# EDIpack/EDIpack

Measured on AMD Instinct MI355X. Metric: Lanczos H*v iterations/sec, largest (Nup,Ndw) sector, higher is better.
Workload: dtype f64

## Files before the change

edipack_amd/csrc/edigpu_capi.hip:

```cpp
#include <algorithm>
#include <chrono>
#include <cmath>
#include <cstdlib>
#include <cstring>
#include <map>
#include <memory>
#include <mutex>
#include <tuple>

#include "host_ib.hpp"
#include "host_sb.hpp"
#include "kernels.hpp"

namespace edigpu {

static thread_local std::string g_err;
static thread_local int g_device = 0;
void set_error(const std::string& msg) { g_err = msg; }

template <class T>
static int dev_upload(T** d, const T* h, size_t n) {
  *d = nullptr;
  if (n == 0) return 0;
  EDIGPU_HIP(hipMalloc((void**)d, n * sizeof(T)));
  EDIGPU_HIP(hipMemcpy(*d, h, n * sizeof(T), hipMemcpyHostToDevice));
  return 0;
}

template <class T>
static void dev_free(T*& p) {
  if (p) (void)hipFree(p);
  p = nullptr;
}

static int ensure_device(int* count_out = nullptr) {
  int n = 0;
  hipError_t e = hipGetDeviceCount(&n);
  if (e != hipSuccess || n <= 0) {
    set_error(std::string("edigpu: no usable HIP device (") +
              (e != hipSuccess ? hipGetErrorString(e) : "device count 0") +
              "); this library has no CPU fallback");
    if (count_out) *count_out = 0;
    return 1;
  }
  if (count_out) *count_out = n;
  return 0;
}

static int upload_csr(DevCsr& d, int64_t nrow, const int64_t* rowptr, const int32_t* col,
                      const double* val, int cplx) {
  d = DevCsr();
  d.nrow = nrow;
  d.nnz = rowptr ? rowptr[nrow] : 0;
  d.avg_row = nrow > 0 ? (double)d.nnz / (double)nrow : 0.0;
  if (nrow == 0) return 0;
  if (d.nnz >= ((int64_t)1 << 31)) {
    d.wide = 1;
    if (dev_upload(&d.rowptr64, rowptr, (size_t)nrow + 1)) return 1;
  } else {
    std::vector<int32_t> rp((size_t)nrow + 1);
    for (int64_t i = 0; i <= nrow; i++) rp[i] = (int32_t)rowptr[i];
    if (dev_upload(&d.rowptr32, rp.data(), rp.size())) return 1;
  }
  std::vector<int32_t> cpad(col, col + d.nnz);
  cpad.resize((size_t)d.nnz + 8, 0);
  std::vector<double> vpad(val, val + (size_t)d.nnz * (cplx ? 2 : 1));
  vpad.resize(vpad.size() + 8, 0.0);
  if (dev_upload(&d.col, cpad.data(), cpad.size())) return 1;
  if (dev_upload(&d.val, vpad.data(), vpad.size())) return 1;
  return 0;
}

static void free_ell(DevEll& e) {
  dev_free(e.pk);
  dev_free(e.coef);
  dev_free(e.col);
  dev_free(e.val);
}

static void free_csr(DevCsr& d) {
  dev_free(d.sell_ptr);
  dev_free(d.sell_pk);
  dev_free(d.sell_dict);
  dev_free(d.sell_diag);
  dev_free(d.sell_col);
  dev_free(d.sell_val);
  dev_free(d.rowptr32);
  dev_free(d.rowptr64);
  dev_free(d.col);
  dev_free(d.val);
}

static int upload_ell(DevEll& e, const HostCsr& a, bool lds) {
  e = DevEll();
  const uint32_t cmul = lds ? 8u : 1u;
  e.nrow = a.nrow;
  e.pitch = (a.nrow + 63) / 64 * 64;
  int w = 0;
  for (int64_t i = 0; i < a.nrow; i++) w = std::max<int>(w, (int)(a.rowptr[i + 1] - a.rowptr[i]));
  e.width = w;
  if (w == 0 || a.nrow == 0) return 0;
  std::vector<double> coef(1, 0.0);
  bool packable = (a.nrow + 1) * (int64_t)cmul < ((int64_t)1 << 24);
  std::vector<uint8_t> cid((size_t)a.nnz());
  for (int64_t p = 0; p < a.nnz() && packable; p++) {
    const double m = std::fabs(a.val[p]);
    size_t k = 0;
    for (; k < coef.size(); k++)
      if (coef[k] == m) break;
    if (k == coef.size()) {
      if (coef.size() >= 128) {
        packable = false;
        break;
      }
      coef.push_back(m);
    }
    cid[p] = (uint8_t)k;
  }
  bool typed = packable && coef.size() > 1 && !getenv("EDIGPU_ELL_UNTYPED");
  std::vector<int> maxmult(coef.size(), 0), base(coef.size() + 1, 0);
  if (typed) {
    std::vector<int> cnt(coef.size());
    for (int64_t i = 0; i < a.nrow; i++) {
      std::fill(cnt.begin(), cnt.end(), 0);
      for (int64_t p = a.rowptr[i]; p < a.rowptr[i + 1]; p++) cnt[cid[p]]++;
      for (size_t v = 1; v < coef.size(); v++) maxmult[v] = std::max(maxmult[v], cnt[v]);
    }
    for (size_t v = 1; v < coef.size(); v++) base[v + 1] = base[v] + maxmult[v];
    const int nt = base[coef.size()];
    typed = nt >= 1 && nt <= 127 && nt <= std::max(2 * w, w + 8);
  }
  if (typed) {
    const int nt = base[coef.size()];
    e.width = nt;
    e.typed = 1;
    std::vector<double> tc(128, 0.0);
    for (size_t v = 1; v < coef.size(); v++)
      for (int j = 0; j < maxmult[v]; j++) tc[base[v] + j] = coef[v];
    std::vector<uint32_t> pk((size_t)nt * e.pitch, lds ? (uint32_t)a.nrow * 8u : 0u);
    std::vector<int> occ(coef.size());
    for (int64_t i = 0; i < a.nrow; i++) {
      std::fill(occ.begin(), occ.end(), 0);
      for (int64_t p = a.rowptr[i]; p < a.rowptr[i + 1]; p++) {
        if (cid[p] == 0) continue;
        const int slot = base[cid[p]] + occ[cid[p]]++;
        pk[(size_t)slot * e.pitch + i] = (uint32_t)a.col[p] * cmul | (lds ? 0u : 1u << 24) |
                                         (std::signbit(a.val[p]) ? 0x80000000u : 0u);
      }
    }
    if (dev_upload(&e.pk, pk.data(), pk.size())) return 1;
    if (dev_upload(&e.coef, tc.data(), tc.size())) return 1;
    return 0;
  }
  if (packable) {
    coef.resize(128, 0.0);
    std::vector<uint32_t> pk((size_t)w * e.pitch);
    for (int k = 0; k < w; k++)
      for (int64_t i = 0; i < e.pitch; i++) pk[(size_t)k * e.pitch + i] = (uint32_t)std::min(i, a.nrow - 1) * cmul;
    for (int64_t i = 0; i < a.nrow; i++) {
      int k = 0;
      for (int64_t p = a.rowptr[i]; p < a.rowptr[i + 1]; p++, k++)
        pk[(size_t)k * e.pitch + i] = (uint32_t)a.col[p] * cmul | ((uint32_t)cid[p] << 24) |
                                      (std::signbit(a.val[p]) ? 0x80000000u : 0u);
    }
    if (dev_upload(&e.pk, pk.data(), pk.size())) return 1;
    if (dev_upload(&e.coef, coef.data(), coef.size())) return 1;
    return 0;
  }
  std::vector<int32_t> col((size_t)w * e.pitch);
  std::vector<double> val((size_t)w * e.pitch, 0.0);
  for (int k = 0; k < w; k++)
    for (int64_t i = 0; i < e.pitch; i++) col[(size_t)k * e.pitch + i] = (int32_t)std::min(i, a.nrow - 1);
  for (int64_t i = 0; i < a.nrow; i++) {
    int k = 0;
    for (int64_t p = a.rowptr[i]; p < a.rowptr[i + 1]; p++, k++) {
      col[(size_t)k * e.pitch + i] = a.col[p];
      val[(size_t)k * e.pitch + i] = a.val[p];
    }
  }
  if (dev_upload(&e.col, col.data(), col.size())) return 1;
  if (dev_upload(&e.val, val.data(), val.size())) return 1;
  return 0;
}

static int upload_sell(DevCsr& d, int64_t nrow, int64_t ncol, const int64_t* rowptr, const int32_t* col,
                       const double* val, int cplx, bool is_loc, double max_pad = 1.6) {
  if (nrow == 0 || rowptr[nrow] == 0 || getenv("EDIGPU_CSR_NOSELL")) return 0;
  const int w = cplx ? 2 : 1;
  bool packed = ncol < ((int64_t)1 << 24) && !getenv("EDIGPU_CSR_UNPACKED");
  std::vector<double> dict(w, 0.0);
  std::vector<uint8_t> ids;
  std::vector<double> diag;
  if (packed) {
    ids.assign((size_t)rowptr[nrow], 0);
    if (is_loc) diag.assign((size_t)nrow * w, 0.0);
    for (int64_t i = 0; i < nrow && packed; i++)
      for (int64_t k = rowptr[i]; k < rowptr[i + 1]; k++) {
        if (is_loc && col[k] == i) {
          for (int q = 0; q < w; q++) diag[i * w + q] += val[k * w + q];
          continue;
        }
        const size_t n = dict.size() / w;
        size_t id = 0;
        for (; id < n; id++)
// ... 433 lines not shown
      dst.rimg_len = src.rimg_len;
      for (int i = 0; i < 5; i++) {
        dst.ucls[i] = src.ucls[std::min(i, h.norb + 1)];
        dst.rcb[i] = src.rcb[i];
        dst.rcs[i] = src.rcs[i];
      }
      std::vector<uint32_t> m2((size_t)src.npanels * kIbPanel / 2);
      for (size_t i = 0; i < m2.size(); i++) m2[i] = (uint32_t)src.rmap[2 * i] | ((uint32_t)src.rmap[2 * i + 1] << 16);
      rc = dev_upload(&dst.ublist, src.ublist.data(), src.ublist.size()) || dev_upload(&dst.utop, src.utop.data(), src.utop.size()) ||
           dev_upload(&dst.rmap2, m2.data(), m2.size());
    }
    if (rc) {
      free_ib(p);
      return 1;
    }
  }
  s->ib = d.release();
  if (setup_sb(s->ib, hn, h, chunk_rows)) return 1;
  return setup_pos_rows(s, hn, h);
}

static int setup_normal(edigpu_sector* s, int64_t dim_up, int64_t dim_dw, int64_t dw_first,
                        int64_t dw_count, const double* hd, const HostCsr& up, const HostCsr& dw,
                        const int64_t* nd_rowptr, const int32_t* nd_col, const double* nd_val,
                        HostNormal* built = nullptr) {
  s->kind = 0;
  s->is_complex = 0;
  s->device = g_device;
  s->dim_up = dim_up;
  s->dim_dw = dim_dw;
  s->dw_first = dw_first;
  s->dw_count = dw_count;
  s->dim = dim_up * dim_dw;
  s->nloc = dim_up * dw_count;
  s->row_first = dw_first * dim_up;
  s->h_up = up;
  s->h_dw = dw;
  std::vector<int32_t> tile_starts;
  s->rows_per_block = normal_pick_rows_per_block(dim_up, dw_count);
  {
    const char* e = getenv("EDIGPU_ROW_SPLIT");
    int parts = 0;
    if (e) {
      parts = atoi(e);
      if (parts > 1) s->rows_per_block = 0;
    } else if (s->rows_per_block == 0) {
      parts = (int)(((dim_up + 2) * 8 + 140 * 1024 - 1) / (140 * 1024));
    }
    if (s->rows_per_block == 0 && parts > 1 && dim_up >= 4 * parts) {
      if (upload_ell(s->up_ell, up, true)) return 1;
      if (s->up_ell.typed && s->up_ell.pk) {
        s->row_split = parts;
      } else {
        dev_free(s->up_ell.pk);
        dev_free(s->up_ell.coef);
        dev_free(s->up_ell.col);
        dev_free(s->up_ell.val);
      }
    }
  }
  if (s->row_split == 1 && upload_ell(s->up_ell, up, s->rows_per_block != 0)) return 1;
  if (upload_csr(s->dw, dim_dw, dw.rowptr.data(), dw.col.data(), dw.val.data(), 0)) return 1;
  for (int64_t i = 0; i < dim_dw; i++)
    s->dw_maxrow = std::max<int>(s->dw_maxrow, (int)(dw.rowptr[i + 1] - dw.rowptr[i]));
  {
    const char* e;
    const bool vec2_env = !(e = getenv("EDIGPU_PANEL_VEC2")) || atoi(e) != 0;
    const int64_t vec2_min = (e = getenv("EDIGPU_PANEL_VEC2_MIN")) ? atoll(e) : ((int64_t)1 << 21);
    const bool tile_env = !(e = getenv("EDIGPU_PANEL_TILE")) || atoi(e) != 0;
    int rmax = (e = getenv("EDIGPU_TILE_ROWS")) ? atoi(e) : 32;
    if (rmax < 8) rmax = 8;
    if (rmax > 64) rmax = 64;
    if (vec2_env && dim_up >= 2 && dim_up * dw_count >= vec2_min) s->panel_mode = 1;
    if (s->panel_mode == 1 && tile_env && dw_count > 0 && dim_dw < ((int64_t)1 << 24)) {
      std::vector<int32_t> starts;
      plan_tile_chunks(dw, dw_first, dw_count, rmax, starts, s->tile_rows);
      s->tile_nchunks = (int)starts.size() - 1;
      if (dev_upload(&s->d_tile_chunks, starts.data(), starts.size())) return 1;
      tile_starts = starts;
      s->panel_mode = 2;
    }
  }
  s->has_nd = nd_rowptr != nullptr && nd_rowptr[s->nloc] > 0;
  s->nd_nnz = s->has_nd ? nd_rowptr[s->nloc] : 0;
  if (built && !nd_rowptr) {
    s->has_nd = built->has_nd && built->nd_nnz > 0;
    s->nd_nnz = s->has_nd ? built->nd_nnz : 0;
  }
  if (built && built->fac.valid && built->fac.nterms <= 16 && !env_flag("EDIGPU_NORMAL_EXPLICIT")) {
    const HostFactored& f = built->fac;
    s->factored = 1;
    s->fac_nimp = f.nimp;
    s->fac_nterms = f.nterms;
    if (dev_upload(&s->d_eux, f.eux.data(), f.eux.size())) return 1;
    if (dev_upload(&s->d_ed, f.ed.data(), f.ed.size())) return 1;
    if (dev_upload(&s->d_impd, f.impd.data(), f.impd.size())) return 1;
    if (f.nterms > 0) {
      if (dev_upload(&s->d_ndcoef, f.coef.data(), f.coef.size())) return 1;
      if (dev_upload(&s->d_jup, f.jup.data(), f.jup.size())) return 1;
      for (int t = 0; t < f.nterms; t++)
        for (int64_t c = 0; c < dim_up; c++) {
          const uint32_t jt = f.jup[(size_t)t * dim_up + c];
          if (jt != 0xFFFFFFFFu)
            s->col_halo = std::max<int>(s->col_halo, (int)std::llabs((int64_t)(jt & 0x7FFFFFFFu) - c));
        }
      if (dev_upload(&s->d_jdw, f.jdw.data(), f.jdw.size())) return 1;
      if (dim_dw < ((int64_t)1 << 24) && f.nterms < 127) {
        std::vector<int32_t> mp((size_t)dw_count + 1, 0), mc;
        std::vector<double> mv;
        for (int64_t r = 0; r < dw_count; r++) {
// ... 2537 lines not shown
    float ms = 0.f;
    rc |= (hipEventElapsedTime(&ms, ev[2 * k], ev[2 * k + 1]) != hipSuccess);
    hv += ms;
  }
  for (auto& e : ev) (void)hipEventDestroy(e);
  if (rc) {
    if (g_err.empty()) set_error("edigpu_lanczos_bench: HIP failure");
    return 1;
  }
  *ms_wall_per_step = std::chrono::duration<double, std::milli>(t1 - t0).count() / steps;
  *ms_hv_per_launch = hv / steps;
  return 0;
}

int edigpu_destroy(edigpu_handle s) {
  if (!s) return 0;
  (void)hipSetDevice(s->device);
  if (s->stream) {
    (void)hipStreamSynchronize(s->stream);
    (void)hipStreamDestroy(s->stream);
  }
  if (s->sub_s) edigpu_destroy(s->sub_s);
  if (s->sub_a) edigpu_destroy(s->sub_a);
  if (s->sub_d) edigpu_destroy(s->sub_d);
  dev_free(s->d_cz);
  dev_free(s->d_hd);
  dev_free(s->d_gu);
  dev_free(s->d_gd);
  dev_free(s->d_mx_rowptr);
  dev_free(s->d_tile_chunks);
  dev_free(s->d_tile_lbeg);
  if (s->lz_graph) (void)hipGraphExecDestroy(s->lz_graph);
  dev_free(s->d_lzcnt);
  dev_free(s->d_bl_meta);
  dev_free(s->d_bl_lend);
  dev_free(s->d_bl_ent);
  dev_free(s->d_bl_wtab);
  if (s->ib) {
    free_ib(s->ib);
    delete s->ib;
    s->ib = nullptr;
  }
  dev_free(s->d_tl_meta);
  dev_free(s->d_tl_col);
  dev_free(s->d_tl_val);
  dev_free(s->d_mx_col);
  dev_free(s->d_mx_val);
  dev_free(s->d_eux);
  dev_free(s->d_ed);
  dev_free(s->d_impd);
  dev_free(s->d_ndcoef);
  dev_free(s->d_jup);
  dev_free(s->d_jdw);
  dev_free(s->up_ell.pk);
  dev_free(s->up_ell.coef);
  dev_free(s->up_ell.col);
  dev_free(s->up_ell.val);
  free_csr(s->dw);
  free_csr(s->nd);
  free_csr(s->loc);
  free_csr(s->nonloc);
  for (const void* q : {(const void*)s->orbs.ell_col, (const void*)s->orbs.ell_val, (const void*)s->orbs.hd,
                        (const void*)s->orbs.eax, (const void*)s->orbs.impbit, (const void*)s->orbs.xtab})
    if (q) (void)hipFree(const_cast<void*>(q));
  s->orbs = OrbsArgs();
  dev_free(s->d_dir_states);
  dev_free(s->d_dir_offdw);
  dev_free(s->d_dir_rkup);
  dev_free(s->d_dir_terms);
  dev_free(s->d_dir_tests);
  dev_free(s->d_dir_dtab);
  dev_free(s->d_dir_xtab);
  dev_free(s->d_vin);
  dev_free(s->d_vout);
  dev_free(s->d_tmp);
  dev_free(s->d_partial);
  dev_free(s->d_scal);
  delete s;
  return 0;
}

}
```

edipack_amd/csrc/edigpu_internal.hpp:

```cpp
#pragma once
#include <hip/hip_runtime.h>

#include <cstdint>
#include <cstdio>
#include <string>
#include <vector>

#include "../../include/edigpu.h"
#include "host_build.hpp"

namespace edigpu {

void set_error(const std::string& msg);

#define EDIGPU_HIP(call)                                                                     \
  do {                                                                                       \
    hipError_t _e = (call);                                                                  \
    if (_e != hipSuccess) {                                                                  \
      ::edigpu::set_error(std::string(#call) + " failed: " + hipGetErrorString(_e) + " (" +  \
                          __FILE__ + ":" + std::to_string(__LINE__) + ")");                  \
      return 1;                                                                              \
    }                                                                                        \
  } while (0)

struct DevCsr {
  int64_t nrow = 0, nnz = 0;
  int wide = 0;
  int32_t* rowptr32 = nullptr;
  int64_t* rowptr64 = nullptr;
  int32_t* col = nullptr;
  double* val = nullptr;
  double avg_row = 0.0;
  int sell = 0;
  int64_t nslice = 0;
  int32_t* sell_ptr = nullptr;
  int32_t* sell_col = nullptr;
  double* sell_val = nullptr;
  int sell_packed = 0;
  uint32_t* sell_pk = nullptr;
  double* sell_dict = nullptr;
  double* sell_diag = nullptr;
};

constexpr int kOrbsMaxAxes = 2 * EDIGPU_MAXORB;
struct OrbsArgs {
  int naxes = 0;
  int64_t dim = 0;
  int64_t dims[kOrbsMaxAxes] = {0};
  int64_t stride[kOrbsMaxAxes] = {0};
  int off[kOrbsMaxAxes] = {0};
  int width[kOrbsMaxAxes] = {0};
  int64_t elloff[kOrbsMaxAxes] = {0};
  const int32_t* ell_col = nullptr;
  const double* ell_val = nullptr;
  const double* hd = nullptr;
  const double* eax = nullptr;
  const uint8_t* impbit = nullptr;
  const double* xtab = nullptr;
};

struct DevEll {
  int64_t nrow = 0, pitch = 0;
  int width = 0;
  int typed = 0;
  uint32_t* pk = nullptr;
  double* coef = nullptr;
  int32_t* col = nullptr;
  double* val = nullptr;
};

struct IbDevHalf {
  int panel0 = 0, npanels = 0, nlist = 0, rimg_len = 0;
  int ucls[5] = {0, 0, 0, 0, 0}, rcb[5] = {0, 0, 0, 0, 0}, rcs[5] = {0, 0, 0, 0, 0};
  uint16_t *ublist = nullptr, *utop = nullptr;
  uint32_t* rmap2 = nullptr;
};

struct DevSb {
  int nb0 = 0, nloc = 0, amode = 0, nbw_up = 0, nbw_dw = 0;
  int rows_nt = 0, rows_nbt = 0, rimg_len = 0, rcs = 0;
  size_t rows_lds = 0, cols_lds = 0;
  uint16_t *urank = nullptr, *ublist = nullptr;
  double* ebw = nullptr;
  int32_t* uslot = nullptr;
  uint32_t* rmap2 = nullptr;
  double *up_vtab = nullptr, *up_tloc = nullptr, *e0 = nullptr;
  uint32_t* up_korb = nullptr;
  int lowbits = 0, nchunks = 0, max_chunk_rows = 0, max_chunk_slots = 0, cols_gs = 8;
  int32_t *chunk_row = nullptr, *chunk_slot = nullptr, *cdesc_off = nullptr;
  uint8_t* cdesc = nullptr;
  double *dw_vtab = nullptr, *dw_tloc = nullptr;
  uint32_t* dw_korb = nullptr;
  uint32_t* nd_dw = nullptr;
  int nhalf = 1;
  struct Half {
    int panel0 = 0, npanels = 0;
    uint32_t* ublist32 = nullptr;
    uint8_t* ugap = nullptr;
    int32_t* uslot = nullptr;
    uint32_t* rmap2 = nullptr;
    double* ebw = nullptr;
  } half[2];
};

struct IbDev {
  DevSb* sb = nullptr;
  int nhalf = 1;
  IbDevHalf half[2];
  uint16_t* urank_low = nullptr;
  double top_eps = 0.0;
  int norb = 0, nb_up = 0, nb_dw = 0, npanels = 0, plen = 0, nlist = 0;
  int ucls[5] = {0, 0, 0, 0, 0};
  int lowbits = 0, nchunks = 0, max_chunk_rows = 0, max_chunk_blocks = 0, nterms = 0, nsub = 1;
  int64_t dim_up = 0, dim_dw = 0, ps = 0, len = 0;
  int rows_nt = 0, rows_nbt = 0;
  size_t rows_lds = 0, cols_lds = 0;
  uint16_t *urank = nullptr, *ublist = nullptr;
  uint32_t* rmap2 = nullptr;
  int rcb[5] = {0, 0, 0, 0, 0}, rcs[5] = {0, 0, 0, 0, 0}, rimg_len = 0;
// ... 114 lines not shown
```

edipack_amd/csrc/kernels_normal.hip:

```cpp
#include <cstdlib>
#include <string>

#include "kernels.hpp"
#include "normal_args.hpp"

namespace edigpu {



constexpr int kE = 4;

template <bool VEC>
__device__ inline void load4(const double* __restrict__ base, int64_t i0, const bool* ok, double* out) {
  if (VEC) {
    const double2 a = ok[0] ? *reinterpret_cast<const double2*>(base + i0) : make_double2(0.0, 0.0);
    const double2 b = ok[2] ? *reinterpret_cast<const double2*>(base + i0 + 2) : make_double2(0.0, 0.0);
    out[0] = a.x;
    out[1] = a.y;
    out[2] = b.x;
    out[3] = b.y;
  } else {
#pragma unroll
    for (int e = 0; e < kE; e++) out[e] = ok[e] ? base[i0 + e] : 0.0;
  }
}

typedef const double __attribute__((address_space(3))) lds_cdouble;
__device__ inline double lds_abs_read(uint32_t byte_addr) { return *reinterpret_cast<lds_cdouble*>(byte_addr); }

template <int NT, int TD, bool USE_LDS, bool LOCAL, bool ND, bool PACKED, bool VEC, bool HDF, int FUSE,
          bool SPLIT = false>
__global__ void __launch_bounds__(NT)
    normal_rows_kernel(NormalArgs a, const double* v_local, const double* __restrict__ v_full,
                       double* hv) {
  extern __shared__ double vs[];

  const int64_t DimUp = a.dim_up;
  const int bsh = a.blk_shift;
  const int64_t bps = a.blk_ps;
  auto vix = [&](int64_t row, int64_t col) -> int64_t {
    return bsh ? (col >> bsh) * bps + (row << bsh) + (col & (((int64_t)1 << bsh) - 1)) : row * DimUp + col;
  };
  const int64_t sf = SPLIT ? a.split_first : 0, sc = SPLIT ? a.split_count : DimUp;
  const int S = ((int)sc + 2) & ~1;
  const int rowB = S * 8;
  double* coef_s = vs + (USE_LDS ? TD * S : 0);
  const int64_t r0 = (int64_t)blockIdx.x * TD;
  const int tid = threadIdx.x;
  int nr = TD;
  if (r0 + nr > a.dw_count) nr = (int)(a.dw_count - r0);
  double beta = 0.0, ibeta = 1.0;
  if (FUSE != 0) {
    if (a.scal[SC_STOP] != 0.0) return;
    if (FUSE >= 2) {
      beta = a.scal[SC_BETA];
      ibeta = 1.0 / beta;
    }
  }
  const double alpha = (FUSE == 3) ? a.scal[SC_ALPHA] : 0.0;
  const double* __restrict__ v_src = (FUSE >= 2) ? hv : v_local;

  if (LOCAL && PACKED && tid < 128) coef_s[tid] = a.ell_coef[tid];
  if (LOCAL && USE_LDS) {
    if ((uint32_t)(uintptr_t)(__attribute__((address_space(3))) double*)vs != 0u) __builtin_trap();
    if (tid < TD) vs[tid * S + sc] = 0.0;
    if (VEC) {
      const int64_t n2 = sc >> 1;
      for (int64_t j0 = 0; j0 < n2; j0 += 4 * NT) {
        double2 t[TD][4];
#pragma unroll
        for (int r = 0; r < TD; r++)
#pragma unroll
          for (int u = 0; u < 4; u++) {
            const int64_t j = j0 + tid + u * NT;
            const int rr = r < nr ? r : 0;
            const int64_t jc = 2 * (j < n2 ? j : n2 - 1);
            t[r][u] = *reinterpret_cast<const double2*>(v_src + vix(r0 + rr, sf + jc));
            if (FUSE == 3) {
              const double2 pp = *reinterpret_cast<const double2*>(v_local + vix(r0 + rr, jc));
              t[r][u].x -= alpha * pp.x;
              t[r][u].y -= alpha * pp.y;
            }
            if (FUSE >= 2) {
              t[r][u].x *= ibeta;
              t[r][u].y *= ibeta;
            }
          }
#pragma unroll
        for (int r = 0; r < TD; r++)
#pragma unroll
          for (int u = 0; u < 4; u++) {
            const int64_t j = j0 + tid + u * NT;
            if (r < nr && j < n2) reinterpret_cast<double2*>(vs + r * S)[j] = t[r][u];
          }
      }
    } else {
      for (int64_t j0 = 0; j0 < sc; j0 += 4 * NT) {
        double t[TD][4];
#pragma unroll
        for (int r = 0; r < TD; r++)
#pragma unroll
          for (int u = 0; u < 4; u++) {
            const int64_t j = j0 + tid + u * NT;
            const int rr = r < nr ? r : 0;
            t[r][u] = v_src[vix(r0 + rr, sf + (j < sc ? j : sc - 1))];
            if (FUSE == 3) t[r][u] -= alpha * v_local[vix(r0 + rr, j < DimUp ? j : DimUp - 1)];
            if (FUSE >= 2) t[r][u] *= ibeta;
          }
#pragma unroll
        for (int r = 0; r < TD; r++)
#pragma unroll
          for (int u = 0; u < 4; u++) {
            const int64_t j = j0 + tid + u * NT;
            if (r < nr && j < sc) vs[r * S + j] = t[r][u];
          }
      }
    }
  }
  __syncthreads();

  for (int64_t c0 = 0; c0 < DimUp; c0 += (int64_t)NT * kE) {
    const int64_t col0 = c0 + (int64_t)tid * kE;
    if (col0 >= DimUp) break;
    double acc[TD][kE];
    bool ok[kE];
#pragma unroll
    for (int e = 0; e < kE; e++) {
      ok[e] = col0 + e < DimUp;
#pragma unroll
      for (int r = 0; r < TD; r++) acc[r][e] = 0.0;
    }

    if (LOCAL) {
#pragma unroll
      for (int r = 0; r < TD; r++)
        if (r < nr) {
          double h[kE], x[kE];
          if (HDF) {
            const int64_t g = a.dw_first + r0 + r;
            const double edr = a.ed[g];
            load4<VEC>(a.eux, (int64_t)a.impd[g] * DimUp + col0, ok, h);
#pragma unroll
            for (int e = 0; e < kE; e++) h[e] += edr;
          } else {
            load4<VEC>(a.hd, (r0 + r) * DimUp + col0, ok, h);
          }
          if (USE_LDS && !SPLIT) {
#pragma unroll
            for (int e = 0; e < kE; e++) x[e] = ok[e] ? vs[r * S + col0 + e] : 0.0;
          } else {
            load4<VEC>(v_local, vix(r0 + r, col0), ok, x);
          }
#pragma unroll
          for (int e = 0; e < kE; e++) acc[r][e] = (SPLIT && sf != 0) ? 0.0 : h[e] * x[e];
        }
      constexpr int KU = 4;
      const bool fast = PACKED && USE_LDS && a.ell_typed != 0;
      if (fast) {
        const uint32_t* __restrict__ epk = a.ell_pk + col0;
        const int epitch = (int)a.ell_pitch;
        for (int k0 = 0; k0 < a.ell_w; k0 += KU) {
          uint4 pk4[KU];
          double tk[KU];
#pragma unroll
          for (int u = 0; u < KU; u++) {
            const int k = k0 + u < a.ell_w ? k0 + u : a.ell_w - 1;
            pk4[u] = *reinterpret_cast<const uint4*>(epk + k * epitch);
            tk[u] = coef_s[k0 + u < 127 ? k0 + u : 127];
          }
#pragma unroll
          for (int u = 0; u < KU; u++) {
            const uint32_t p[kE] = {pk4[u].x, pk4[u].y, pk4[u].z, pk4[u].w};
#pragma unroll
            for (int r = 0; r < TD; r++)
              if (TD == 1 || r < nr) {
#pragma unroll
                for (int e = 0; e < kE; e++) {
                  uint32_t off = p[e] & 0xFFFFFFu;
                  if (SPLIT) {
                    const uint32_t rel = off - (uint32_t)(sf * 8);
                    off = rel < (uint32_t)(sc * 8) ? rel : (uint32_t)(sc * 8);
                  }
                  double x = lds_abs_read((uint32_t)(r * rowB) + off);
                  x = __hiloint2double(__double2hiint(x) ^ (int)(p[e] & 0x80000000u), __double2loint(x));
                  acc[r][e] = fma(tk[u], x, acc[r][e]);
                }
              }
          }
        }
      }
      for (int k0 = fast ? a.ell_w : 0; k0 < a.ell_w; k0 += KU) {
        uint4 pk4[KU];
        int4 pc4[KU];
        double2 pw0[KU], pw1[KU];
#pragma unroll
        for (int u = 0; u < KU; u++) {
          const int k = k0 + u < a.ell_w ? k0 + u : a.ell_w - 1;
          const int64_t o = (int64_t)k * a.ell_pitch + col0;
          if (PACKED) {
            pk4[u] = *reinterpret_cast<const uint4*>(a.ell_pk + o);
          } else {
            pc4[u] = *reinterpret_cast<const int4*>(a.ell_col + o);
            pw0[u] = *reinterpret_cast<const double2*>(a.ell_val + o);
            pw1[u] = *reinterpret_cast<const double2*>(a.ell_val + o + 2);
          }
        }
#pragma unroll
        for (int u = 0; u < KU; u++) {
          const bool live = k0 + u < a.ell_w;
          int32_t cc[kE];
          double ww[kE];
          if (PACKED) {
            const uint32_t p[kE] = {pk4[u].x, pk4[u].y, pk4[u].z, pk4[u].w};
            if (a.ell_typed) {
              const double tk = live ? coef_s[k0 + u] : 0.0;
              if (USE_LDS) {
#pragma unroll
                for (int e = 0; e < kE; e++) {
                  cc[e] = (int32_t)(p[e] & 0xFFFFFFu);
                  ww[e] = __hiloint2double(__double2hiint(tk) ^ (int)(p[e] & 0x80000000u), __double2loint(tk));
                }
              } else {
#pragma unroll
                for (int e = 0; e < kE; e++) {
                  cc[e] = (int32_t)(p[e] & 0xFFFFFFu);
                  const double m = ((p[e] >> 24) & 0x7Fu) ? tk : 0.0;
                  ww[e] = (p[e] >> 31) ? -m : m;
                }
              }
            } else {
#pragma unroll
              for (int e = 0; e < kE; e++) {
                cc[e] = (int32_t)(p[e] & 0xFFFFFFu);
                const double m = live ? coef_s[(p[e] >> 24) & 0x7Fu] : 0.0;
                ww[e] = (p[e] >> 31) ? -m : m;
              }
            }
          } else {
            cc[0] = pc4[u].x; cc[1] = pc4[u].y; cc[2] = pc4[u].z; cc[3] = pc4[u].w;
            ww[0] = live ? pw0[u].x : 0.0; ww[1] = live ? pw0[u].y : 0.0;
            ww[2] = live ? pw1[u].x : 0.0; ww[3] = live ? pw1[u].y : 0.0;
          }
#pragma unroll
          for (int r = 0; r < TD; r++)
            if (r < nr) {
#pragma unroll
              for (int e = 0; e < kE; e++) {
                const double x = USE_LDS ? (PACKED ? *reinterpret_cast<const double*>(
                                                         reinterpret_cast<const char*>(vs) + r * rowB + cc[e])
                                                   : vs[r * S + cc[e]])
                                         : v_local[vix(r0 + r, cc[e])];
                acc[r][e] = fma(ww[e], x, acc[r][e]);
              }
            }
        }
      }
    }
    if (ND) {
      if (a.has_nd) {
        int64_t rp[TD][kE + 1];
#pragma unroll
        for (int r = 0; r < TD; r++)
          if (r < nr) {
            const int64_t i0 = (r0 + r) * DimUp + col0;
#pragma unroll
            for (int e = 0; e <= kE; e++) {
              const int64_t i = (e == 0 || ok[e - 1]) ? i0 + e : i0;
              rp[r][e] = a.nd_rp64 ? a.nd_rp64[i] : (int64_t)a.nd_rp32[i];
            }
          }
#pragma unroll
        for (int r = 0; r < TD; r++)
          if (r < nr) {
#pragma unroll
            for (int e = 0; e < kE; e++)
              if (ok[e]) {
                double s = 0.0;
                for (int64_t jj = rp[r][e]; jj < rp[r][e + 1]; jj++)
                  s += a.nd_val[jj] * v_full[a.nd_col[jj]];
                acc[r][e] += s;
              }
          }
      }
    }
#pragma unroll
    for (int r = 0; r < TD; r++)
      if (r < nr) {
        double* dst = hv + vix(r0 + r, col0);
        if (!LOCAL || (SPLIT && sf != 0)) {
          double old[kE];
          load4<VEC>(hv, vix(r0 + r, col0), ok, old);
#pragma unroll
          for (int e = 0; e < kE; e++) acc[r][e] += old[e];
        }
        if (FUSE >= 2) {
          double pold[kE];
          load4<VEC>(v_local, vix(r0 + r, col0), ok, pold);
          double* pdst = (a.xout ? a.xout : const_cast<double*>(v_local)) + vix(r0 + r, col0);
#pragma unroll
          for (int e = 0; e < kE; e++) acc[r][e] -= beta * pold[e];
          if (VEC) {
            if (ok[0]) *reinterpret_cast<double2*>(pdst) = make_double2(vs[r * S + col0], vs[r * S + col0 + 1]);
            if (ok[2]) *reinterpret_cast<double2*>(pdst + 2) = make_double2(vs[r * S + col0 + 2], vs[r * S + col0 + 3]);
          } else {
#pragma unroll
            for (int e = 0; e < kE; e++)
              if (ok[e]) pdst[e] = vs[r * S + col0 + e];
          }
        }
        if (VEC) {
          if (ok[0]) *reinterpret_cast<double2*>(dst) = make_double2(acc[r][0], acc[r][1]);
          if (ok[2]) *reinterpret_cast<double2*>(dst + 2) = make_double2(acc[r][2], acc[r][3]);
        } else {
#pragma unroll
          for (int e = 0; e < kE; e++)
            if (ok[e]) dst[e] = acc[r][e];
        }
      }
  }
}

int normal_pick_rows_per_block(int64_t dim_up, int64_t dw_count) {
  const int64_t row_bytes = ((dim_up + 2) & ~(int64_t)1) * 8;
  if (const char* e = getenv("EDIGPU_ROWS_TD")) {
    const int td = atoi(e);
    if ((td == 1 || td == 2 || td == 4 || td == 8) && td * row_bytes <= 150 * 1024) return td;
  }
  if (row_bytes > 150 * 1024) return 0;
  int td = 1;
  for (int cand : {2, 4, 8}) {
    if (cand * row_bytes > 24 * 1024) break;
    if ((dw_count + cand - 1) / cand < 1024) break;
    td = cand;
  }
  return td;
}

template <int NT, int TD, bool USE_LDS, bool PACKED, bool VEC, bool HDF>
static int launch_te(const NormalArgs& a, const double* vl, const double* vf, double* hv,
                     int what, hipStream_t st) {
  const int64_t nblk = (a.dw_count + TD - 1) / TD;
  const size_t lds = (USE_LDS ? (size_t)TD * ((a.dim_up + 2) & ~(int64_t)1) * sizeof(double) : 0) + 128 * sizeof(double);
  dim3 grid((unsigned)nblk), block(NT);
#define EDIGPU_LAUNCH_ROWS(LOC, NDF, LDSB, UL, PK, HF)                                           \
  do {                                                                                           \
    auto kern = normal_rows_kernel<NT, TD, UL, LOC, NDF, PK, VEC, HF, 0>;                            \
    if (ensure_dynamic_lds((const void*)kern, (LDSB))) return 1; \
    hipLaunchKernelGGL(kern, grid, block, (LDSB), st, a, vl, vf, hv);                            \
  } while (0)
  switch (what) {
    case 1: EDIGPU_LAUNCH_ROWS(true, false, lds, USE_LDS, PACKED, HDF); break;
    case 5: EDIGPU_LAUNCH_ROWS(true, true, lds, USE_LDS, PACKED, HDF); break;
    case 101: {
      auto kern = normal_rows_kernel<NT, TD, USE_LDS, true, false, PACKED, VEC, HDF, 1>;
      if (ensure_dynamic_lds((const void*)kern, lds)) return 1;
      hipLaunchKernelGGL(kern, grid, block, lds, st, a, vl, vf, hv);
      break;
    }
    case 102: {
      auto kern = normal_rows_kernel<NT, TD, USE_LDS, true, false, PACKED, VEC, HDF, 2>;
      if (ensure_dynamic_lds((const void*)kern, lds)) return 1;
      hipLaunchKernelGGL(kern, grid, block, lds, st, a, vl, vf, hv);
      break;
    }
    case 103: {
      auto kern = normal_rows_kernel<NT, TD, USE_LDS, true, false, PACKED, VEC, HDF, 3>;
      if (ensure_dynamic_lds((const void*)kern, lds)) return 1;
      hipLaunchKernelGGL(kern, grid, block, lds, st, a, vl, vf, hv);
      break;
    }
    case 4: EDIGPU_LAUNCH_ROWS(false, true, (size_t)0, false, false, false); break;
    default: set_error("launch_normal: bad term mask"); return 1;
  }
#undef EDIGPU_LAUNCH_ROWS
  EDIGPU_HIP(hipGetLastError());
  return 0;
}

template <int TD, bool USE_LDS>
static int launch_td(const NormalArgs& a, bool packed, bool hdf, const double* vl, const double* vf,
                     double* hv, int what, hipStream_t st) {
  const bool vec = (a.dim_up % 2) == 0;
  const bool big = TD == 1 && USE_LDS && (size_t)a.dim_up * sizeof(double) > 80 * 1024;
  constexpr int NTBIG = (TD == 1 && USE_LDS) ? 1024 : 512;
#define EDIGPU_TD(PK, VC)                                                                  \
  (big ? (hdf ? launch_te<NTBIG, TD, USE_LDS, PK, VC, true>(a, vl, vf, hv, what, st)       \
              : launch_te<NTBIG, TD, USE_LDS, PK, VC, false>(a, vl, vf, hv, what, st))     \
       : (hdf ? launch_te<512, TD, USE_LDS, PK, VC, true>(a, vl, vf, hv, what, st)         \
              : launch_te<512, TD, USE_LDS, PK, VC, false>(a, vl, vf, hv, what, st)))
  if (vec) return packed ? EDIGPU_TD(true, true) : EDIGPU_TD(false, true);
  return packed ? EDIGPU_TD(true, false) : EDIGPU_TD(false, false);
#undef EDIGPU_TD
}

template <bool VEC, bool HDF>
static int launch_split_t(const edigpu_sector* s, NormalArgs a, const double* vl, double* hv, hipStream_t st) {
  constexpr int NT = 1024;
  const int64_t part = (((a.dim_up + s->row_split - 1) / s->row_split) + 1) & ~(int64_t)1;
  auto kern = normal_rows_kernel<NT, 1, true, true, false, true, VEC, HDF, 0, true>;
  const size_t lds = (size_t)((part + 2) & ~(int64_t)1) * sizeof(double) + 128 * sizeof(double);
  if (ensure_dynamic_lds((const void*)kern, lds)) return 1;
  for (int64_t first = 0; first < a.dim_up; first += part) {
    a.split_first = first;
    a.split_count = std::min<int64_t>(part, a.dim_up - first);
    hipLaunchKernelGGL(kern, dim3((unsigned)a.dw_count), dim3(NT), lds, st, a, vl, nullptr, hv);
  }
  EDIGPU_HIP(hipGetLastError());
  return 0;
}

static int launch_rows(const edigpu_sector* s, const NormalArgs& a, const double* vl,
                       const double* vf, double* hv, int what, hipStream_t st) {
  const bool packed = s->up_ell.pk != nullptr;
  const bool hdf = s->factored != 0;
  if (s->row_split > 1 && what != 4) {
    if (what != 1 && what != 5) {
      set_error("launch_normal: fused Lanczos is not available for split rows");
      return 1;
    }
    const bool vec = (a.dim_up % 2) == 0;
    const int rc = vec ? (hdf ? launch_split_t<true, true>(s, a, vl, hv, st) : launch_split_t<true, false>(s, a, vl, hv, st))
                       : (hdf ? launch_split_t<false, true>(s, a, vl, hv, st) : launch_split_t<false, false>(s, a, vl, hv, st));
    if (rc || what == 1) return rc;
    return launch_td<1, false>(a, false, hdf, vl, vf, hv, 4, st);
  }
  switch (s->rows_per_block) {
    case 0: return launch_td<1, false>(a, packed, hdf, vl, vf, hv, what, st);
    case 1: return launch_td<1, true>(a, packed, hdf, vl, vf, hv, what, st);
    case 2: return launch_td<2, true>(a, packed, hdf, vl, vf, hv, what, st);
    case 4: return launch_td<4, true>(a, packed, hdf, vl, vf, hv, what, st);
    case 8: return launch_td<8, true>(a, packed, hdf, vl, vf, hv, what, st);
    default: set_error("launch_normal: bad rows_per_block"); return 1;
  }
}

static void fill_args(const edigpu_sector* s, NormalArgs& a) {
  a.dim_up = s->dim_up;
  a.dim_dw = s->dim_dw;
  a.dw_first = s->dw_first;
  a.dw_count = s->dw_count;
  a.hd = s->d_hd;
  a.eux = s->d_eux;
  a.ed = s->d_ed;
  a.impd = s->d_impd;
  a.ell_pk = s->up_ell.pk;
  a.ell_coef = s->up_ell.coef;
  a.ell_col = s->up_ell.col;
  a.ell_val = s->up_ell.val;
  a.ell_w = s->up_ell.width;
  a.ell_typed = s->up_ell.typed;
  a.ell_pitch = s->up_ell.pitch;
  a.dw_rowptr = s->dw.rowptr32;
  a.dw_col = s->dw.col;
  a.dw_val = s->dw.val;
  a.dw_maxrow = s->dw_maxrow;
  a.nd_rp32 = s->nd.rowptr32;
  a.nd_rp64 = s->nd.wide ? s->nd.rowptr64 : nullptr;
  a.nd_col = s->nd.col;
  a.nd_val = s->nd.val;
  a.has_nd = s->has_nd;
  a.nterms = s->factored ? s->fac_nterms : 0;
  a.nd_coef = s->d_ndcoef;
  a.jup = s->d_jup;
  a.jdw = s->d_jdw;
  a.panel_mode = s->panel_mode;
  a.tile_nchunks = s->tile_nchunks;
  a.tile_rows = s->tile_rows;
  a.tile_chunks = s->d_tile_chunks;
  a.tile_lbeg = s->d_tile_lbeg;
  a.tile_list_cap = s->tile_list_cap;
  a.tl_meta = s->d_tl_meta;
  a.tl_col = s->d_tl_col;
  a.tl_val = s->d_tl_val;
  a.tl_has_nd = s->tl_has_nd;
  a.blk_shift = 0;
  a.blk_ps = 0;
  a.bl_meta = s->d_bl_meta;
  a.blk_rows = s->blk_rows;
  a.blk_list_cap = s->blk_list_cap;
  a.bl_lend = s->d_bl_lend;
  a.bl_ent = s->d_bl_ent;
  a.bl_wtab = s->d_bl_wtab;
  a.mx_rowptr = s->d_mx_rowptr;
  a.mx_col = s->d_mx_col;
  a.mx_val = s->d_mx_val;
  a.scal = nullptr;
  a.partial = nullptr;
  a.xout = nullptr;
  a.partial_cap = 0;
  a.lz_counter = nullptr;
  a.lz_nlanc = 0;
  a.lz_len = 0;
  a.split_first = 0;
  a.split_count = s->dim_up;
}

int launch_normal(const edigpu_sector* s, const double* v_local, const double* v_full, double* hv,
                  int phase, hipStream_t st) {
  NormalArgs a;
  fill_args(s, a);
  if (s->dw_count == 0) return 0;
  const bool fac = s->factored != 0;
  const bool sell_nd = !fac && s->has_nd && s->nd.sell;
  const bool csr_nd = !fac && s->has_nd && !sell_nd;
  const bool fac_nd = fac && a.nterms > 0 && s->d_mx_rowptr != nullptr;
  if (phase == 1) return launch_rows(s, a, v_local, v_full, hv, 1, st);
  if (phase == 3) {
    if (launch_rows(s, a, v_local, v_full, hv, csr_nd ? 5 : 1, st)) return 1;
    if (launch_dw_panels(a, true, fac_nd, v_full, hv, st)) return 1;
    return sell_nd ? launch_csr(s->nd, 0, v_full, hv, 1, st) : 0;
  }
  if (csr_nd && launch_rows(s, a, v_local, v_full, hv, 4, st)) return 1;
  if (launch_dw_panels(a, true, fac_nd, v_full, hv, st)) return 1;
  return sell_nd ? launch_csr(s->nd, 0, v_full, hv, 1, st) : 0;
}

int launch_normal_rows_pos(const edigpu_sector* s, const double* P, double* Q, double* X, int what, const double* scal, hipStream_t st) {
  const IbDev* d = s->ib;
  NormalArgs a;
  fill_args(s, a);
  a.dim_up = d->plen;
  a.split_count = d->plen;
  a.eux = d->pr.eux;
  a.ell_pk = d->pr.ell.pk;
  a.ell_coef = d->pr.ell.coef;
  a.ell_col = d->pr.ell.col;
  a.ell_val = d->pr.ell.val;
  a.ell_w = d->pr.ell.width;
  a.ell_typed = d->pr.ell.typed;
  a.ell_pitch = d->pr.ell.pitch;
  a.blk_shift = 4;
  a.blk_ps = d->ps;
  a.scal = scal;
  a.xout = X;
  const bool packed = d->pr.ell.pk != nullptr;
  switch (d->pr.td) {
    case 1: return launch_td<1, true>(a, packed, true, P, P, Q, what, st);
    case 2: return launch_td<2, true>(a, packed, true, P, P, Q, what, st);
    case 4: return launch_td<4, true>(a, packed, true, P, P, Q, what, st);
    case 8: return launch_td<8, true>(a, packed, true, P, P, Q, what, st);
  }
  set_error("launch_normal_rows_pos: rows per workgroup");
  return 1;
}

bool normal_transposable_el(const edigpu_sector* s) {
  if (s->kind != 0 || s->nloc != s->dim || s->dw_count == 0) return false;
  if (!s->factored && s->has_nd) return false;
  if (s->factored && s->fac_nterms > 0 && s->d_mx_rowptr == nullptr) return false;
  return true;
}

bool normal_transposable(const edigpu_sector* s) { return s->nph == 0 && normal_transposable_el(s); }

int launch_normal_rows(const edigpu_sector* s, int64_t dw_first, int64_t dw_count, const double* v_rows,
                       double* hv_rows, hipStream_t st) {
  if (dw_count <= 0) return 0;
  NormalArgs a;
  fill_args(s, a);
  a.dw_first = dw_first;
  a.dw_count = dw_count;
  return launch_rows(s, a, v_rows, nullptr, hv_rows, 1, st);
}

int launch_normal_cols(const edigpu_sector* s, int64_t col_first, int64_t ncol, int64_t stride, int halo,
                       const double* w, double* hv, hipStream_t st) {
  NormalArgs a;
  fill_args(s, a);
  const bool fac_nd = s->factored && a.nterms > 0;
  return launch_dw_panel_cols(a, fac_nd, col_first, ncol, stride, halo, w, hv, st);
}

bool normal_lanczos_fusable(const edigpu_sector* s) {
  if (s->kind != 0 || s->nloc != s->dim || s->dw_count == 0 || s->nph > 0) return false;
  if (s->rows_per_block == 0) return false;
  if (!s->factored && s->has_nd && !s->nd.sell) return false;
  if (getenv("EDIGPU_LANCZOS_UNFUSED")) return false;
// ... 60 lines not shown
```

edipack_amd/csrc/normal_args.hpp:

```cpp
#pragma once
#include <cstdint>

#include "kernels.hpp"

namespace edigpu {

struct NormalArgs {
  int64_t dim_up, dim_dw, dw_first, dw_count;
  const double* hd;
  const double* eux;
  const double* ed;
  const uint8_t* impd;
  const uint32_t* ell_pk;
  const double* ell_coef;
  const int32_t* ell_col;
  const double* ell_val;
  int ell_w;
  int ell_typed;
  int64_t split_first, split_count;
  int64_t ell_pitch;
  const int32_t* dw_rowptr;
  const int32_t* dw_col;
  const double* dw_val;
  const int32_t* nd_rp32;
  const int64_t* nd_rp64;
  const int32_t* nd_col;
  const double* nd_val;
  int dw_maxrow;
  int has_nd;
  int nterms;
  const double* nd_coef;
  const uint32_t* jup;
  const uint32_t* jdw;
  const double* scal;
  double* partial;
  double* xout;
  int64_t partial_cap;
  unsigned int* lz_counter;
  int lz_nlanc;
  int64_t lz_len;
  int panel_mode;
  int tile_nchunks, tile_rows;
  const int32_t* tile_chunks;
  const int32_t* tile_lbeg;
  int tile_list_cap;
  const int4* tl_meta;
  const int32_t* tl_col;
  const double* tl_val;
  int tl_has_nd;
  int blk_shift;
  int64_t blk_ps;
  const int4* bl_meta;
  const uint32_t* bl_ent;
  int blk_rows;
  int blk_list_cap;
  const int32_t* bl_lend;
  const double* bl_wtab;
  const int32_t* mx_rowptr;
  const int32_t* mx_col;
  const double* mx_val;
};

int launch_dw_panels(const NormalArgs& a, bool do_dw, bool do_nd, const double* v_full, double* hv,
                     hipStream_t st, bool alpha = false, int* nblocks = nullptr);

int launch_dw_blocked(const NormalArgs& a, bool do_nd, const double* v, double* hv, hipStream_t st, bool alpha,
                      int* nblocks);
// ... 6 lines not shown
```

Before: 6370.

## Pack typed ELL up-hop entries into 16-bit halves and keep p vector in registers

Adds a second copy of the typed ELL index array in which each entry is squeezed into 16 bits (15-bit LDS byte offset plus sign), two entries per word. The row kernel gets a path that reads this packed array when the up-dimension fits in LDS, halving index traffic. A second variant for the fused Lanczos step (FUSE==3, one row per block) loads the old vector once into registers at staging time and reuses it for the beta subtraction instead of reloading from global memory. This adds extra device memory for the packed copy, more template instantiations and register pressure. The ELL free paths are also consolidated into free_ell.

After: 6746, median of 6. 1.06x the previous value.

```diff
diff --git a/edipack_amd/csrc/edigpu_capi.hip b/edipack_amd/csrc/edigpu_capi.hip
--- a/edipack_amd/csrc/edigpu_capi.hip
+++ b/edipack_amd/csrc/edigpu_capi.hip
@@ -73,6 +73,7 @@
 
 static void free_ell(DevEll& e) {
   dev_free(e.pk);
+  dev_free(e.pk16);
   dev_free(e.coef);
   dev_free(e.col);
   dev_free(e.val);
@@ -150,6 +151,20 @@
     }
     if (dev_upload(&e.pk, pk.data(), pk.size())) return 1;
     if (dev_upload(&e.coef, tc.data(), tc.size())) return 1;
+    const char* e16 = getenv("EDIGPU_ELL16");
+    if (lds && (uint64_t)a.nrow * 8u <= 0x7FFFu && !(e16 && atoi(e16) == 0)) {
+      const uint32_t dead = (uint32_t)a.nrow * 8u;
+      const int np = (nt + 1) / 2;
+      std::vector<uint32_t> pk16((size_t)np * e.pitch, dead | dead << 16);
+      for (int k = 0; k < nt; k++)
+        for (int64_t i = 0; i < a.nrow; i++) {
+          const uint32_t p = pk[(size_t)k * e.pitch + i];
+          const uint32_t h = (p & 0x7FFFu) | (p >> 31) << 15;
+          uint32_t& wd = pk16[(size_t)(k >> 1) * e.pitch + i];
+          wd = (k & 1) ? (wd & 0xFFFFu) | h << 16 : (wd & 0xFFFF0000u) | h;
+        }
+      if (dev_upload(&e.pk16, pk16.data(), pk16.size())) return 1;
+    }
     return 0;
   }
   if (packable) {
@@ -689,10 +704,8 @@
       if (s->up_ell.typed && s->up_ell.pk) {
         s->row_split = parts;
       } else {
-        dev_free(s->up_ell.pk);
-        dev_free(s->up_ell.coef);
-        dev_free(s->up_ell.col);
-        dev_free(s->up_ell.val);
+        free_ell(s->up_ell);
+        s->up_ell = DevEll();
       }
     }
   }
@@ -3336,10 +3349,7 @@
   dev_free(s->d_ndcoef);
   dev_free(s->d_jup);
   dev_free(s->d_jdw);
-  dev_free(s->up_ell.pk);
-  dev_free(s->up_ell.coef);
-  dev_free(s->up_ell.col);
-  dev_free(s->up_ell.val);
+  free_ell(s->up_ell);
   free_csr(s->dw);
   free_csr(s->nd);
   free_csr(s->loc);
diff --git a/edipack_amd/csrc/edigpu_internal.hpp b/edipack_amd/csrc/edigpu_internal.hpp
--- a/edipack_amd/csrc/edigpu_internal.hpp
+++ b/edipack_amd/csrc/edigpu_internal.hpp
@@ -65,6 +65,7 @@
   int typed = 0;
   uint32_t* pk = nullptr;
   double* coef = nullptr;
+  uint32_t* pk16 = nullptr;
   int32_t* col = nullptr;
   double* val = nullptr;
 };
diff --git a/edipack_amd/csrc/kernels_normal.hip b/edipack_amd/csrc/kernels_normal.hip
--- a/edipack_amd/csrc/kernels_normal.hip
+++ b/edipack_amd/csrc/kernels_normal.hip
@@ -29,7 +29,7 @@
 __device__ inline double lds_abs_read(uint32_t byte_addr) { return *reinterpret_cast<lds_cdouble*>(byte_addr); }
 
 template <int NT, int TD, bool USE_LDS, bool LOCAL, bool ND, bool PACKED, bool VEC, bool HDF, int FUSE,
-          bool SPLIT = false>
+          bool SPLIT = false, bool E16 = false, bool KP = false>
 __global__ void __launch_bounds__(NT)
     normal_rows_kernel(NormalArgs a, const double* v_local, const double* __restrict__ v_full,
                        double* hv) {
@@ -60,8 +60,38 @@
   const double alpha = (FUSE == 3) ? a.scal[SC_ALPHA] : 0.0;
   const double* __restrict__ v_src = (FUSE >= 2) ? hv : v_local;
 
+  constexpr bool KEEPP = KP && FUSE == 3 && TD == 1 && USE_LDS && LOCAL && !SPLIT;
+  double pkeep[2][kE];
+
   if (LOCAL && PACKED && tid < 128) coef_s[tid] = a.ell_coef[tid];
-  if (LOCAL && USE_LDS) {
+  if (KEEPP) {
+    if ((uint32_t)(uintptr_t)(__attribute__((address_space(3))) double*)vs != 0u) __builtin_trap();
+    if (tid == 0) vs[sc] = 0.0;
+#pragma unroll
+    for (int ps = 0; ps < 2; ps++) {
+      const int64_t col0 = (int64_t)ps * NT * kE + (int64_t)tid * kE;
+      bool ok[kE];
+#pragma unroll
+      for (int e = 0; e < kE; e++) ok[e] = col0 + e < DimUp;
+      const int64_t cs = ok[0] ? col0 : 0;
+      double q[kE];
+      load4<VEC>(v_src, vix(r0, cs), ok, q);
+      load4<VEC>(v_local, vix(r0, cs), ok, pkeep[ps]);
+#pragma unroll
+      for (int e = 0; e < kE; e++) {
+        q[e] -= alpha * pkeep[ps][e];
+        q[e] *= ibeta;
+      }
+      if (VEC) {
+        if (ok[0]) *reinterpret_cast<double2*>(vs + col0) = make_double2(q[0], q[1]);
+        if (ok[2]) *reinterpret_cast<double2*>(vs + col0 + 2) = make_double2(q[2], q[3]);
+      } else {
+#pragma unroll
+        for (int e = 0; e < kE; e++)
+          if (ok[e]) vs[col0 + e] = q[e];
+      }
+    }
+  } else if (LOCAL && USE_LDS) {
     if ((uint32_t)(uintptr_t)(__attribute__((address_space(3))) double*)vs != 0u) __builtin_trap();
     if (tid < TD) vs[tid * S + sc] = 0.0;
     if (VEC) {
@@ -156,7 +186,39 @@
         }
       constexpr int KU = 4;
       const bool fast = PACKED && USE_LDS && a.ell_typed != 0;
-      if (fast) {
+      if (E16) {
+        const uint32_t* __restrict__ epk = a.ell_pk16 + col0;
+        const int epitch = (int)a.ell_pitch;
+        const int np = (a.ell_w + 1) >> 1;
+        constexpr int KU = KEEPP ? 2 : 4;
+        for (int k0 = 0; k0 < a.ell_w; k0 += KU) {
+          uint4 pk2[KU / 2];
+          double tk[KU];
+#pragma unroll
+          for (int u = 0; u < KU / 2; u++) {
+            const int q = (k0 >> 1) + u < np ? (k0 >> 1) + u : np - 1;
+            pk2[u] = *reinterpret_cast<const uint4*>(epk + q * epitch);
+          }
+#pragma unroll
+          for (int u = 0; u < KU; u++) tk[u] = coef_s[k0 + u < 127 ? k0 + u : 127];
+#pragma unroll
+          for (int u = 0; u < KU; u++) {
+            const uint32_t p[kE] = {pk2[u >> 1].x, pk2[u >> 1].y, pk2[u >> 1].z, pk2[u >> 1].w};
+#pragma unroll
+            for (int r = 0; r < TD; r++)
+              if (TD == 1 || r < nr) {
+#pragma unroll
+                for (int e = 0; e < kE; e++) {
+                  const uint32_t off = (u & 1) ? (p[e] >> 16) & 0x7FFFu : p[e] & 0x7FFFu;
+                  const uint32_t sgn = (u & 1) ? p[e] & 0x80000000u : (p[e] & 0x8000u) << 16;
+                  double x = lds_abs_read((uint32_t)(r * rowB) + off);
+                  x = __hiloint2double(__double2hiint(x) ^ (int)sgn, __double2loint(x));
+                  acc[r][e] = fma(tk[u], x, acc[r][e]);
+                }
+              }
+          }
+        }
+      } else if (fast) {
         const uint32_t* __restrict__ epk = a.ell_pk + col0;
         const int epitch = (int)a.ell_pitch;
         for (int k0 = 0; k0 < a.ell_w; k0 += KU) {
@@ -189,7 +251,7 @@
           }
         }
       }
-      for (int k0 = fast ? a.ell_w : 0; k0 < a.ell_w; k0 += KU) {
+      for (int k0 = (E16 || fast) ? a.ell_w : 0; k0 < a.ell_w; k0 += KU) {
         uint4 pk4[KU];
         int4 pc4[KU];
         double2 pw0[KU], pw1[KU];
@@ -295,7 +357,12 @@
         }
         if (FUSE >= 2) {
           double pold[kE];
-          load4<VEC>(v_local, vix(r0 + r, col0), ok, pold);
+          if (KEEPP) {
+#pragma unroll
+            for (int e = 0; e < kE; e++) pold[e] = c0 == 0 ? pkeep[0][e] : pkeep[1][e];
+          } else {
+            load4<VEC>(v_local, vix(r0 + r, col0), ok, pold);
+          }
           double* pdst = (a.xout ? a.xout : const_cast<double*>(v_local)) + vix(r0 + r, col0);
 #pragma unroll
           for (int e = 0; e < kE; e++) acc[r][e] -= beta * pold[e];
@@ -336,7 +403,7 @@
   return td;
 }
 
-template <int NT, int TD, bool USE_LDS, bool PACKED, bool VEC, bool HDF>
+template <int NT, int TD, bool USE_LDS, bool PACKED, bool VEC, bool HDF, bool E16>
 static int launch_te(const NormalArgs& a, const double* vl, const double* vf, double* hv,
                      int what, hipStream_t st) {
   const int64_t nblk = (a.dw_count + TD - 1) / TD;
@@ -344,7 +411,7 @@
   dim3 grid((unsigned)nblk), block(NT);
 #define EDIGPU_LAUNCH_ROWS(LOC, NDF, LDSB, UL, PK, HF)                                           \
   do {                                                                                           \
-    auto kern = normal_rows_kernel<NT, TD, UL, LOC, NDF, PK, VEC, HF, 0>;                            \
+    auto kern = normal_rows_kernel<NT, TD, UL, LOC, NDF, PK, VEC, HF, 0, false, E16 && LOC>;     \
     if (ensure_dynamic_lds((const void*)kern, (LDSB))) return 1; \
     hipLaunchKernelGGL(kern, grid, block, (LDSB), st, a, vl, vf, hv);                            \
   } while (0)
@@ -352,19 +419,26 @@
     case 1: EDIGPU_LAUNCH_ROWS(true, false, lds, USE_LDS, PACKED, HDF); break;
     case 5: EDIGPU_LAUNCH_ROWS(true, true, lds, USE_LDS, PACKED, HDF); break;
     case 101: {
-      auto kern = normal_rows_kernel<NT, TD, USE_LDS, true, false, PACKED, VEC, HDF, 1>;
+      auto kern = normal_rows_kernel<NT, TD, USE_LDS, true, false, PACKED, VEC, HDF, 1, false, E16>;
       if (ensure_dynamic_lds((const void*)kern, lds)) return 1;
       hipLaunchKernelGGL(kern, grid, block, lds, st, a, vl, vf, hv);
       break;
     }
     case 102: {
-      auto kern = normal_rows_kernel<NT, TD, USE_LDS, true, false, PACKED, VEC, HDF, 2>;
+      auto kern = normal_rows_kernel<NT, TD, USE_LDS, true, false, PACKED, VEC, HDF, 2, false, E16>;
       if (ensure_dynamic_lds((const void*)kern, lds)) return 1;
       hipLaunchKernelGGL(kern, grid, block, lds, st, a, vl, vf, hv);
       break;
     }
     case 103: {
-      auto kern = normal_rows_kernel<NT, TD, USE_LDS, true, false, PACKED, VEC, HDF, 3>;
+      constexpr bool kp_ok = E16 && TD == 1 && NT == 512 && USE_LDS && PACKED;
+      if (kp_ok && a.dim_up <= 2 * NT * kE) {
+        auto kern = normal_rows_kernel<NT, TD, USE_LDS, true, false, PACKED, VEC, HDF, 3, false, E16, kp_ok>;
+        if (ensure_dynamic_lds((const void*)kern, lds)) return 1;
+        hipLaunchKernelGGL(kern, grid, block, lds, st, a, vl, vf, hv);
+        break;
+      }
+      auto kern = normal_rows_kernel<NT, TD, USE_LDS, true, false, PACKED, VEC, HDF, 3, false, E16>;
       if (ensure_dynamic_lds((const void*)kern, lds)) return 1;
       hipLaunchKernelGGL(kern, grid, block, lds, st, a, vl, vf, hv);
       break;
@@ -383,11 +457,14 @@
   const bool vec = (a.dim_up % 2) == 0;
   const bool big = TD == 1 && USE_LDS && (size_t)a.dim_up * sizeof(double) > 80 * 1024;
   constexpr int NTBIG = (TD == 1 && USE_LDS) ? 1024 : 512;
-#define EDIGPU_TD(PK, VC)                                                                  \
-  (big ? (hdf ? launch_te<NTBIG, TD, USE_LDS, PK, VC, true>(a, vl, vf, hv, what, st)       \
-              : launch_te<NTBIG, TD, USE_LDS, PK, VC, false>(a, vl, vf, hv, what, st))     \
-       : (hdf ? launch_te<512, TD, USE_LDS, PK, VC, true>(a, vl, vf, hv, what, st)         \
-              : launch_te<512, TD, USE_LDS, PK, VC, false>(a, vl, vf, hv, what, st)))
+  const bool e16 = USE_LDS && packed && a.ell_typed != 0 && a.ell_pk16 != nullptr && !big;
+#define EDIGPU_TD(PK, VC)                                                                             \
+  (big   ? (hdf ? launch_te<NTBIG, TD, USE_LDS, PK, VC, true, false>(a, vl, vf, hv, what, st)         \
+                : launch_te<NTBIG, TD, USE_LDS, PK, VC, false, false>(a, vl, vf, hv, what, st))       \
+   : e16 ? (hdf ? launch_te<512, TD, USE_LDS, PK, VC, true, (PK && USE_LDS)>(a, vl, vf, hv, what, st) \
+                : launch_te<512, TD, USE_LDS, PK, VC, false, (PK && USE_LDS)>(a, vl, vf, hv, what, st)) \
+         : (hdf ? launch_te<512, TD, USE_LDS, PK, VC, true, false>(a, vl, vf, hv, what, st)           \
+                : launch_te<512, TD, USE_LDS, PK, VC, false, false>(a, vl, vf, hv, what, st)))
   if (vec) return packed ? EDIGPU_TD(true, true) : EDIGPU_TD(false, true);
   return packed ? EDIGPU_TD(true, false) : EDIGPU_TD(false, false);
 #undef EDIGPU_TD
@@ -444,6 +521,7 @@
   a.ed = s->d_ed;
   a.impd = s->d_impd;
   a.ell_pk = s->up_ell.pk;
+  a.ell_pk16 = s->up_ell.pk16;
   a.ell_coef = s->up_ell.coef;
   a.ell_col = s->up_ell.col;
   a.ell_val = s->up_ell.val;
@@ -523,6 +601,7 @@
   a.split_count = d->plen;
   a.eux = d->pr.eux;
   a.ell_pk = d->pr.ell.pk;
+  a.ell_pk16 = nullptr;
   a.ell_coef = d->pr.ell.coef;
   a.ell_col = d->pr.ell.col;
   a.ell_val = d->pr.ell.val;
diff --git a/edipack_amd/csrc/normal_args.hpp b/edipack_amd/csrc/normal_args.hpp
--- a/edipack_amd/csrc/normal_args.hpp
+++ b/edipack_amd/csrc/normal_args.hpp
@@ -13,6 +13,7 @@
   const uint8_t* impd;
   const uint32_t* ell_pk;
   const double* ell_coef;
+  const uint32_t* ell_pk16;
   const int32_t* ell_col;
   const double* ell_val;
   int ell_w;
```
